# InternRobotics/InternNav

Hardware: AMD Instinct MI355X
Metric: policy steps/sec/node (higher is better)
Workload: dtype bf16

## Files before the change

internnav_amd/csrc/dit_rowchain.hip:

```cpp
#include <type_traits>
#include <utility>

#pragma clang diagnostic ignored "-Winline-asm"

#include "common.h"
#include "kernels.h"

namespace {

typedef float f32x16 __attribute__((ext_vector_type(16)));
typedef unsigned int u32x2 __attribute__((ext_vector_type(2)));
typedef unsigned int u32x4 __attribute__((ext_vector_type(4)));

constexpr int RC_NS = 4, RC_BN = 128, RC_STAGE = RC_BN * 64, RC_D = 384, RC_NT1 = RC_D / RC_BN, RC_KC2 = RC_D / 64;
constexpr size_t RC_LDS = size_t(RC_NS) * RC_STAGE * sizeof(bf16) + 2 * RC_D * sizeof(float);

__device__ __forceinline__ void rc_glds16(const void* base, uint32_t voff, uint32_t lds_byte_addr) {
    asm volatile("s_mov_b32 m0, %0\n\ts_nop 0\n\tglobal_load_lds_dwordx4 %1, %2" ::"s"(lds_byte_addr), "v"(voff), "s"(base) : "memory", "m0");
}

template <int N>
__device__ __forceinline__ void rc_wait_vm() {
    asm volatile("s_waitcnt vmcnt(%0)" ::"n"(N) : "memory");
}
// ... 356 lines not shown
                    for (int h = 0; h < 2; ++h) {
                        unsigned q[2][2];
#pragma unroll
                        for (int i = 0; i < 2; ++i) {
                            q[i][0] = rc_pack2(acc[j][(2 * h + i) * 4], acc[j][(2 * h + i) * 4 + 1]);
                            q[i][1] = rc_pack2(acc[j][(2 * h + i) * 4 + 2], acc[j][(2 * h + i) * 4 + 3]);
                        }
                        const u32x4 o = rc_merge_rows(q[0][0], q[0][1], q[1][0], q[1][1]);
                        *reinterpret_cast<u32x4*>(Cb + crow + nt * 128 + j * 32 + h * 16 + khalf * 8) = o;
                    }
                }
            }
        }
        rc_wait_vm<0>();
    }
}

template <int NW, int KC1, bool HAS2, bool GLU2>
int launch_rowchain(const ina_dit_rowchain_args& p, hipStream_t stream) {
    auto kern = dit_rowchain_kernel<NW, KC1, HAS2, GLU2>;
    static bool attr_done = false;
    if (!attr_done) {
        INA_HIP_CHECK(hipFuncSetAttribute(reinterpret_cast<const void*>(kern), hipFuncAttributeMaxDynamicSharedMemorySize, (int)RC_LDS));
        attr_done = true;
    }
    const double n2 = HAS2 ? (double)p.N2 : 0.0;
    InaProfScope prof(INA_PROF_GEMM, 2.0 * p.M * RC_D * (p.K1 + n2),
                      2.0 * p.M * p.K1 + 2.0 * RC_D * (p.K1 + n2) + 8.0 * p.M * RC_D + (p.H ? 2.0 * p.M * RC_D : 0.0) + 2.0 * p.M * (GLU2 ? n2 / 2 : n2), stream);
    hipLaunchKernelGGL(kern, dim3(p.M / (NW * 32)), dim3(NW * 64), RC_LDS, stream, p);
    INA_HIP_CHECK(hipGetLastError());
    return 0;
}

}

int ina_launch_dit_rowchain(const ina_dit_rowchain_args& p_in, hipStream_t stream) {
    ina_dit_rowchain_args p = p_in;
    if (p.mod_div <= 0) p.mod_div = p.M;
    constexpr int nw = 4;
    INA_REQUIRE(p.A && p.W1 && p.X && p.gamma1, "dit_rowchain: A, W1, X and gamma1 are required");
    INA_REQUIRE(p.K1 == 384 || p.K1 == 1024, "dit_rowchain: K1=%d (built for 384 = attn2.to_out and 1024 = feed_forward.linear_2)", p.K1);
    INA_REQUIRE(p.M > 0 && p.M % (nw * 32) == 0 && p.mod_div % (nw * 32) == 0, "dit_rowchain: M=%d and mod_div=%d must be multiples of the %d-row panel", p.M,
                p.mod_div, nw * 32);
    INA_REQUIRE(p.lda % 8 == 0 && p.ldw1 % 8 == 0 && p.ldx % 4 == 0 && (!p.H || p.ldh % 8 == 0), "dit_rowchain: row strides must keep 16-byte alignment");
    INA_REQUIRE(((uintptr_t)p.A % 16) == 0 && ((uintptr_t)p.W1 % 16) == 0 && ((uintptr_t)p.X % 16) == 0 && ((uintptr_t)p.H % 16) == 0, "dit_rowchain: misaligned pointer");
    INA_REQUIRE((!p.gate && !p.mod_scale2) || p.mod_ld >= RC_D, "dit_rowchain: modulation needs mod_ld >= 384");
    INA_REQUIRE((size_t)384 * p.ldw1 < (1u << 30) && (!p.W2 || (size_t)p.N2 * p.ldw2 < (1u << 30)), "dit_rowchain: weight too large for 32-bit element offsets");
    INA_REQUIRE(p.W2 || !p.seg_stats, "dit_rowchain: seg_stats are statistics of the second GEMM's output rows");
    if (p.W2) {
        INA_REQUIRE(p.C2 && p.N2 > 0 && p.N2 % 128 == 0 && p.ldw2 % 8 == 0 && p.ldc2 % 8 == 0 && ((uintptr_t)p.W2 % 16) == 0 && ((uintptr_t)p.C2 % 16) == 0,
                    "dit_rowchain: second GEMM needs C2, N2 %% 128 == 0 and 16-byte aligned rows (N2=%d)", p.N2);
        INA_REQUIRE(!p.seg_stats || (!p.glu2 && p.N2 % 384 == 0 && ((uintptr_t)p.seg_stats % 8) == 0), "dit_rowchain: seg_stats needs a plain second GEMM with N2 %% 384 == 0 (N2=%d)", p.N2);
        INA_REQUIRE(p.glu2 ? p.K1 == 384 : p.K1 != 384, "dit_rowchain: built pairs are (K1 = 384, SwiGLU second GEMM) and (K1 = 1024, plain second GEMM)");
    }
    ina_prof_set_sub(42);
    if (p.K1 == 384) return !p.W2 ? launch_rowchain<4, 6, false, false>(p, stream) : launch_rowchain<4, 6, true, true>(p, stream);
    return !p.W2 ? launch_rowchain<4, 16, false, false>(p, stream) : launch_rowchain<4, 16, true, false>(p, stream);
}
```

internnav_amd/nextdit.py:

```python
from __future__ import annotations

import math
from typing import Dict

import numpy as np
import torch

from . import ops
from .navdp import IMAGENET_MEAN, IMAGENET_STD, _DecoderLayer, _SeqWorkspace, decoder_layer_postnorm
from .vit_s import DinoV2Encoder, VitWorkspace


def _interleave16(a: torch.Tensor, b: torch.Tensor) -> torch.Tensor:
    n, k = a.shape
    return torch.stack([a.view(n // 16, 16, k), b.view(n // 16, 16, k)], dim=1).reshape(2 * n, k).contiguous()


class NextDiTSystem1:
    def __init__(self, state_dict: Dict[str, torch.Tensor], cfg: dict, device="cuda:0", max_envs: int = 64, use_async: bool = True, row_chain: bool = True):
        dev = torch.device(device)
        bf, f32 = torch.bfloat16, torch.float32
        sd = state_dict
        self.cfg, self.device, self.b_max = cfg, dev, max_envs
        self.row_chain = (bool(row_chain) and cfg["dit_dim"] == 384 and cfg["dit_ffn"] in (1024, 1536)
                          and (cfg["sample_num"] * cfg["predict_size"]) % 128 == 0)
        self.chain_min_rows = 16384
        self.chain_a, self.chain_b = True, cfg["dit_ffn"] <= 1024
        self.chain_stats = True
        D, L, S, T = cfg["dit_dim"], cfg["latent_dim"], cfg["sample_num"], cfg["predict_size"]
        self.D, self.L, self.S, self.T, self.nq = D, L, S, T, cfg["n_query"]
        self.Fr = cfg["memory_frames"]
        self.use_async = bool(use_async)
        self.Lz = (32 if self.use_async else 0) + self.nq
        self.nl, self.nh = cfg["dit_layers"], cfg["dit_heads"]

        def w(k):
            return sd[k].to(device=dev, dtype=bf).contiguous()

        def f(k):
            return sd[k].to(device=dev, dtype=f32).contiguous()

        self.cp = [(w("cond_projector.0.weight"), f("cond_projector.0.bias")), (w("cond_projector.2.weight"), f("cond_projector.2.bias"))]
        nm = self.Fr * 256
        self.nm = nm
        if self.use_async:
            self.vit = DinoV2Encoder(sd, "rgb_model.", dev)
            self.vit_ws = VitWorkspace(max_envs * self.Fr, dev)
            self.mem_pos = sd["memory_encoder.memory_pos"][:nm].to(device=dev, dtype=f32).contiguous()
        self.me_layers = []
        for i in range(3 if self.use_async else 0):
            p = f"memory_encoder.encoder.layers.{i}"
            self.me_layers.append(dict(sa_w=w(p + ".self_attn.in_proj_weight"), sa_b=f(p + ".self_attn.in_proj_bias"),
                                       sa_ow=w(p + ".self_attn.out_proj.weight"), sa_ob=f(p + ".self_attn.out_proj.bias"),
                                       l1w=w(p + ".linear1.weight"), l1b=f(p + ".linear1.bias"), l2w=w(p + ".linear2.weight"),
                                       l2b=f(p + ".linear2.bias"), n1=(f(p + ".norm1.weight"), f(p + ".norm1.bias")),
                                       n2=(f(p + ".norm2.weight"), f(p + ".norm2.bias"))))
        if self.use_async:
            self.me_ws = _SeqWorkspace(max_envs * nm, D, 2048, dev)
            self.memcat = torch.empty(max_envs * nm, L, dtype=bf, device=dev)
            self.q_layers = [_DecoderLayer(sd, f"rgb_resampler.decoder.layers.{i}", dev, L) for i in range(3)]
# ... 118 lines not shown
        rows = B * nq
        ops.linear(traj_latents.reshape(rows, -1), self.cp[0][0], bias=self.cp[0][1], act="gelu_tanh", out=self.cp_h[:rows])
        ops.linear(self.cp_h[:rows].view(B, nq, L), self.cp[1][0], bias=self.cp[1][1], out=z3[:, Lz - nq:, :], batched=True)
        if self.use_async and not images_encoded:
            self.encode_images(B, images_dp)
        self._derive_condition(B, cs)

    def _derive_condition(self, B: int, cs: dict):
        D, Lz = self.D, self.Lz
        zr = B * Lz
        ops.linear(cs["z"][:zr], self.cap[0][0], bias=self.cap[0][1], act="gelu_tanh", out=cs["cap_h"][:zr])
        ops.linear(cs["cap_h"][:zr], self.cap[1][0], bias=self.cap[1][1], out=cs["enc"][:zr])
        ops.pool_act(cs["enc"][:zr], cs["pool"][:B], T=Lz)
        ops.norm(cs["pool"][:B], self.ce_ln[0], self.ce_ln[1], eps=1e-5, out=cs["pool_n"][:B])
        ops.linear(cs["pool_n"][:B], self.ce_w, bias=self.ce_b, out=cs["cap_emb"][:B])
        for l, Lr in enumerate(self.layers):
            ops.norm(cs["enc"][:zr], Lr["ctx"], None, eps=1e-5, rms=True, out=cs["enc_n"][:zr])
            kv = cs["kv2"][l][:zr]
            ops.linear(cs["enc_n"][:zr], Lr["wkv2"], out=kv)
            kk = kv.view(zr * 2, D)
            ops.norm(kk, Lr["k2n"][0], Lr["k2n"][1], eps=1e-5, out=kk, rows=zr, in_map=(1, 2, 0), out_map=(1, 2, 0))
            ops.dit_v2t(kv.view(B, Lz, 2, self.nh, D // self.nh), self.nh, cs["v2t"][l])

    def _dit_layer(self, l: int, B: int, cs: dict = None, x_buf: torch.Tensor = None):
        Lr, D, S, T, Lz, nh = self.layers[l], self.D, self.S, self.T, self.Lz, self.nh
        cs = cs or self._cond_set()
        rows, nseq, hd = B * S * T, B * S, D // self.nh
        x, h, att, qkvq, proj, ff = (self.x if x_buf is None else x_buf)[:rows], self.h[:rows], self.att[:rows], self.qkvq[:rows], self.proj[:rows], self.ff[:rows]
        mod = cs["mod"]
        m = mod[:B, l * 4 * D:(l + 1) * 4 * D]
        scale_msa, gate_msa, scale_mlp, gate_mlp = m[:, :D], m[:, D:2 * D], m[:, 2 * D:3 * D], m[:, 3 * D:]
        chain = self.row_chain and rows >= self.chain_min_rows
        chain_a, chain_b = chain and self.chain_a, chain and self.chain_b
        stats = self.qstats[:rows] if (chain and self.chain_stats and D == 384) else None
        if l == 0 or not chain_b:
            if l == 0:
                ops.norm(x, Lr["n1"], None, eps=1e-5, rms=True, mod_scale=scale_msa, mod_div=S * T, out=h)
            ops.linear(h, Lr["wq"], out=qkvq, seg_stats=(stats, 1e-5) if stats is not None else None)
        kv5 = cs["kv2"][l][: B * Lz].view(B, Lz, 2, nh, hd)
        ops.dit_attention(qkvq, att, (Lr["q1n"], Lr["k1n"], Lr["q2n"]), kv5, cs["v2t"][l], Lr["gate"], T=T, seq_per_env=S, heads=nh, eps=1e-5, stats=stats)
        last = l + 1 >= self.nl
        nxt = None if last else mod[:B, (l + 1) * 4 * D:(l + 1) * 4 * D + D]
        if chain_a:
            ops.dit_rowchain(att, Lr["wo"], Lr["n2"], x, gate=gate_msa, gamma2=Lr["fn1"], mod_scale2=scale_mlp, w2=Lr["w13"], c2=ff, glu2=True,
                             mod_div=S * T, eps=1e-5)
        else:
            ops.linear(att, Lr["wo"], out=proj)
            ops.norm(proj, Lr["n2"], None, eps=1e-5, rms=True, gate=gate_msa, base=x, mod_div=S * T, out32=x,
                     out2=h, gamma2=Lr["fn1"], mod_scale2=scale_mlp)
            ops.linear(h, Lr["w13"], act="silu", glu=True, out=ff)
        if chain_b:
            if last:
                ops.dit_rowchain(ff, Lr["w2"], Lr["fn2"], x, gate=gate_mlp, mod_div=S * T, eps=1e-5)
            else:
                ops.dit_rowchain(ff, Lr["w2"], Lr["fn2"], x, gate=gate_mlp, gamma2=self.layers[l + 1]["n1"], mod_scale2=nxt,
                                 w2=self.layers[l + 1]["wq"], c2=qkvq, mod_div=S * T, eps=1e-5, seg_stats=stats, seg_eps=1e-5)
            return
        ops.linear(ff, Lr["w2"], out=proj)
        if last:
            ops.norm(proj, Lr["fn2"], None, eps=1e-5, rms=True, gate=gate_mlp, base=x, mod_div=S * T, out32=x)
        else:
            ops.norm(proj, Lr["fn2"], None, eps=1e-5, rms=True, gate=gate_mlp, base=x, mod_div=S * T, out32=x,
                     out2=h, gamma2=self.layers[l + 1]["n1"], mod_scale2=nxt)

    def generate_traj(self, traj_latents: torch.Tensor, images_dp: torch.Tensor, x_init: torch.Tensor, guidance_scale: float = 1.0,
                      images_encoded: bool = False) -> torch.Tensor:
        B = traj_latents.shape[0]
        assert B <= self.b_max and traj_latents.dtype == torch.bfloat16
        D, S, T = self.D, self.S, self.T
        rows = B * S * T
        cs = self._cond_set()
        self.encode_condition(B, traj_latents, images_dp, cs, images_encoded=images_encoded)
        cfg_on = float(guidance_scale) != 1.0
        sets = [(cs, self.x)]
        if cfg_on:
            from . import train_ops as Tr

            null = self._cond_set(null=True)
            self._derive_condition(B, null)
            sets.append((null, self.x_u))
        sample = self.sample[:rows]
        sample.copy_(x_init.reshape(rows, 3))
        nmod = self.nl * 4 * D
        if cfg_on:
            dts = torch.from_numpy(self.sigmas[1:] - self.sigmas[:-1]).float()
            g = float(guidance_scale)
            coefs = torch.stack([dts * g, dts * (1.0 - g)], 1)[:, :, None].expand(-1, -1, 3).contiguous().to(self.device)
        for i in range(self.cfg["num_inference_steps"]):
            dt = float(self.sigmas[i + 1] - self.sigmas[i])
# ... 17 lines not shown
```

internnav_amd/qwen_vl.py:

```python
from __future__ import annotations

import weakref
from types import SimpleNamespace
from typing import Dict, List, Optional, Sequence, Tuple

import numpy as np
import torch

from . import ops
from .runtime import CapacityError


def vision_window_permutation(grids: Sequence[Tuple[int, int, int]], merge: int = 2, window: int = 112, patch: int = 14):
    win = window // merge // patch
    idx_all, cu, base = [], [0], 0
    for t, h, w in grids:
        gh, gw = h // merge, w // merge
        idx = np.arange(t * gh * gw).reshape(t, gh, gw)
        ph, pw = win - gh % win, win - gw % win
        nh, nw = (gh + ph) // win, (gw + pw) // win
        pad = np.pad(idx, ((0, 0), (0, ph), (0, pw)), constant_values=-100)
        pad = pad.reshape(t, nh, win, nw, win).transpose(0, 1, 3, 2, 4).reshape(t, nh * nw, win * win)
        lens = (pad != -100).sum(-1).reshape(-1)
        flat = pad.reshape(-1)
# ... 21 lines not shown

def rope_index(input_ids: np.ndarray, grids, image_token_id: int, vision_start_id: int, merge: int = 2):
    B, S = input_ids.shape
    pos = np.zeros((3, B, S), dtype=np.int64)
    deltas = np.zeros(B, dtype=np.int64)
    img = 0
    for b in range(B):
        toks = input_ids[b]
        starts = np.nonzero((toks[:-1] == vision_start_id) & (toks[1:] == image_token_id))[0]
        chunks, st, nxt = [], 0, 0
        for s0 in starts:
            ed = int(s0) + 1
            t, h, w = grids[img]
            img += 1
            gh, gw = h // merge, w // merge
            text_len = ed - st
            chunks.append(np.broadcast_to(np.arange(text_len)[None], (3, text_len)) + nxt)
            ti = np.zeros(t * gh * gw, dtype=np.int64)
            hi = np.broadcast_to(np.arange(gh)[None, :, None], (t, gh, gw)).reshape(-1)
            wi = np.broadcast_to(np.arange(gw)[None, None, :], (t, gh, gw)).reshape(-1)
            vis = np.stack([ti, hi, wi]) + text_len + nxt
            chunks.append(vis)
            nxt = int(vis.max()) + 1
            st = ed + t * gh * gw
        if st < S:
            chunks.append(np.broadcast_to(np.arange(S - st)[None], (3, S - st)) + nxt)
        p = np.concatenate(chunks, axis=1)
        pos[:, b] = p
        deltas[b] = int(p.max()) + 1 - S
    return pos, deltas


SKINNY_GEMM_MAX_ROWS = 64
ATTN_WIDE_MIN_ROWS = 128


def kv_image_cut(ids: np.ndarray, n: int, image_token_id: int) -> int:
    while 0 < n < ids.shape[0] and ids[n - 1] == image_token_id and ids[n] == image_token_id:
        n -= 1
    return n


def kv_reuse_lengths(ids: np.ndarray, seq_lens, cached_ids: Sequence[Optional[np.ndarray]], image_token_id: int) -> np.ndarray:
    B, S = ids.shape
    lens = np.asarray(seq_lens, dtype=np.int64).reshape(B)
    pl = np.zeros(B, dtype=np.int64)
    for b in range(B):
        c = cached_ids[b]
        if c is None or len(c) == 0:
            continue
        m = min(len(c), int(lens[b]) - 1)
        diff = np.nonzero(ids[b, :m] != np.asarray(c[:m]))[0]
        n = int(diff[0]) if diff.size else m
        pl[b] = kv_image_cut(ids[b], n, image_token_id)
    need = max(ATTN_WIDE_MIN_ROWS, SKINNY_GEMM_MAX_ROWS // B + 1)
    if pl.any() and S - int(pl.min()) < need:
        b = int(np.argmin(pl))
        pl[b] = kv_image_cut(ids[b], max(0, min(int(pl[b]), S - need)), image_token_id)
    return pl


def kv_reuse_fit(pl: np.ndarray, S: int, tail: int, s_max: int) -> Tuple[np.ndarray, int]:
    pl = np.asarray(pl, dtype=np.int64).copy()
    dropped = 0
    while pl.any() and int(pl.max()) + S - int(pl.min()) + tail > s_max:
        pl[int(np.argmax(pl))] = 0
# ... 96 lines not shown
    for k in sd.keys():
        v = sd[k]
        if k in names:
            out[k] = ops.mx4_quantize(v.to(torch.bfloat16).contiguous())[2].to(v.dtype)
        elif k == "lm_head.weight":
            out[k] = ops.w8_quantize(v.to(torch.bfloat16).contiguous())[2].to(v.dtype)
        else:
            out[k] = v
    return out


def _interleave16(a: torch.Tensor, b: torch.Tensor) -> torch.Tensor:
    n, k = a.shape
    return torch.stack([a.view(n // 16, 16, k), b.view(n // 16, 16, k)], dim=1).reshape(2 * n, k).contiguous()


def _pad_rows(t: torch.Tensor, n: int) -> torch.Tensor:
    return t if t.shape[0] == n else torch.cat([t, t.new_zeros((n - t.shape[0],) + tuple(t.shape[1:]))], 0)


class QwenVLEngine:

    def __init__(self, weights, cfg: dict, device="cuda:0", max_seqs: int = 16, max_seq_len: int = 1024, max_patches: int = 16 * 3136,
                 frag_weights: Optional[bool] = None, w8_decode: bool = False, token_logprobs: bool = False, max_decode: int = 128,
                 mx4_decode: bool = False):
        if w8_decode and mx4_decode:
            raise ValueError("w8_decode and mx4_decode are two roundings of the same weights: choose one")
        dev = torch.device(device)
        bf, f32 = torch.bfloat16, torch.float32
        self.cfg, self.device = cfg, dev
        self.B_max, self.S_max, self.Np_max = max_seqs, max_seq_len, max_patches
        self.fuse_decode_norm = True
        self.split_prefill = True
        self.split_serial = False
        self._side = None
        self.fuse_decode_rope = True
        self.tap = None
        D, I = cfg["v_hidden"], cfg["v_inter"]
        Ip = (I + 63) // 64 * 64
        self.vD, self.vI, self.vH, self.vhd = D, Ip, cfg["v_heads"], D // cfg["v_heads"]
        H, TI = cfg["t_hidden"], cfg["t_inter"]
        self.H, self.TI, self.nh, self.nkv = H, TI, cfg["t_heads"], cfg["t_kv_heads"]
        self.hd = H // self.nh
        self.qkv_w = (self.nh + 2 * self.nkv) * self.hd
        self.kv_w = 2 * self.nkv * self.hd
        W = weights

        def w(k):
            return W[k].to(device=dev, dtype=bf).contiguous()

        def f(k):
            return W[k].to(device=dev, dtype=f32).contiguous()

        self.v_patch = W["visual.patch_embed.proj.weight"].to(device=dev, dtype=bf).reshape(D, -1).contiguous()
        self.v_blocks = []
        for i in range(cfg["v_depth"]):
            b = f"visual.blocks.{i}."
            gw_, uw = _pad_rows(W[b + "mlp.gate_proj.weight"].to(dev).float(), Ip), _pad_rows(W[b + "mlp.up_proj.weight"].to(dev).float(), Ip)
            gb, ub = _pad_rows(W[b + "mlp.gate_proj.bias"].to(dev).float(), Ip), _pad_rows(W[b + "mlp.up_proj.bias"].to(dev).float(), Ip)
            dw = W[b + "mlp.down_proj.weight"].to(dev).float()
            dw = torch.cat([dw, dw.new_zeros(D, Ip - I)], 1) if Ip != I else dw
            self.v_blocks.append(dict(
                n1=f(b + "norm1.weight"), n2=f(b + "norm2.weight"), qkv_w=w(b + "attn.qkv.weight"), qkv_b=f(b + "attn.qkv.bias"),
                proj_w=w(b + "attn.proj.weight"), proj_b=f(b + "attn.proj.bias"),
                gu_w=_interleave16(gw_, uw).to(bf), gu_b=_interleave16(gb[:, None], ub[:, None]).reshape(-1).contiguous(),
                down_w=dw.to(bf).contiguous(), down_b=f(b + "mlp.down_proj.bias"), full=i in cfg["v_fullatt"]))
# ... 206 lines not shown
        pos0 = np.broadcast_to(np.asarray(cache_pos0, dtype=np.int64).reshape(-1, 1), (B, 1))
        rows = ((b0 + np.arange(B))[:, None] * self.S_max + pos0 + np.arange(S)[None]).reshape(-1).astype(np.int32)
        if int(pos0.max()) + S > self.S_max:
            raise CapacityError(f"KV cache capacity exceeded: {int(pos0.max()) + S} tokens > max_seq_len={self.S_max}")
        ph = dict(B=B, S=S, pos=torch.from_numpy(np.ascontiguousarray(np.broadcast_to(pos3, (3, B, S)).reshape(3, B * S)).astype(np.int32)).to(dev),
                  rows=torch.from_numpy(rows).to(dev), Lk=int(pos0.max()) + S, k_len=None, b0=b0, r0=b0 * S)
        if k_len is not None:
            ph["k_len"] = torch.from_numpy(np.asarray(k_len, dtype=np.int32)).to(dev)
        ph["new_are_last"] = bool(np.all((np.asarray(k_len).reshape(-1) if k_len is not None else ph["Lk"]) == pos0[:, 0] + S))
        ph["w0"] = pos0[:, 0].copy()
        return ph

    def _layers(self, ph: dict):
        H, nh, nkv, hd, Smax = self.H, self.nh, self.nkv, self.hd, self.S_max
        B, S = ph["B"], ph["S"]
        rows, r0, b0 = B * S, ph.get("r0", 0), ph.get("b0", 0)
        if self._kv_views and "w0" in ph:
            self._kv_evict({b0 + i: int(w) for i, w in enumerate(ph["w0"])})
        x, h, att, qkv, ff, x_in, cos, sin = (t[r0:r0 + rows] for t in (self.x, self.h, self.att, self.qkv, self.ff, self.x_in, self.cos, self.sin))
        ops.mrope_table(ph["pos"], self.inv_freq, self.axis_of, cos, sin)
        q4 = qkv[:, : nh * hd].view(B, S, nh, hd)
        single = rows <= 16 and self.tap is None
        fused_norm = single and self.fuse_decode_norm
        pfx = ph.get("prefix")
        if pfx is not None:
            k4 = qkv[:, nh * hd:(nh + nkv) * hd].view(B, S, nkv, hd)
            v4 = qkv[:, (nh + nkv) * hd:].view(B, S, nkv, hd)
        shr = ph.get("shared")
        fuse_rope = pfx is None and shr is None and single and self.fuse_decode_rope and ph.get("new_are_last", False) and ops.attention_rope_ok(S, ph["Lk"], nh, nkv, hd)
        if fuse_rope:
            kn4 = qkv[:, nh * hd:(nh + nkv) * hd].view(B, S, nkv, hd)
            vn4 = qkv[:, (nh + nkv) * hd:].view(B, S, nkv, hd)
        quant = ("8" if self.w8_decode else "4" if self.mx4_decode else None) if rows <= SKINNY_GEMM_MAX_ROWS else None
        for li, L in enumerate(self.layers):
            src = x_in if li == 0 else x
            wf = (lambda k, L=L: L.get(k)) if (self.frag_weights and rows > SKINNY_GEMM_MAX_ROWS) else (lambda k: None)
            if fused_norm:
                self._linear(src, L, "qkv_w", quant, bias=L["qkv_b"], out=qkv, prenorm=(L["n1"], 1e-6))
            else:
                ops.norm(src, L["n1"], None, eps=1e-6, rms=True, out=h)
                self._linear(h, L, "qkv_w", quant, bias=L["qkv_b"], out=qkv, w_frag=wf("qkv_wf"))
            if pfx is not None:
                ops.rope(qkv, cos, sin, heads=nh + nkv, D=hd, col0=0, rows=rows)
                kvc = L["kv"].view(self.B_max, Smax, 2, nkv, hd)
                tl = pfx.get("tail")
                if tl is None:
                    ops.attention_prefix(q4, k4, v4, kvc[:, :, 0], kvc[:, :, 1], pfx["slot"], pfx["pfx_len"], pfx["suf_len"],
                                         out=att.view(B, S, nh, hd), max_pfx=pfx["max_pfx"])
                else:
                    t5 = tl["tails"][li][: tl["rows"] * tl["T"]].view(tl["rows"], tl["T"], 2, nkv, hd)
                    ops.attention_prefix_tail(q4, k4, v4, kvc[:, :, 0], kvc[:, :, 1], pfx["slot"], pfx["pfx_len"], pfx["suf_len"], t5[:, :, 0],
                                              t5[:, :, 1], tl["tail_row"], tl["tail_len"], out=att.view(B, S, nh, hd), max_pfx=pfx["max_pfx"],
                                              max_tail=tl["max_tail"])
            elif shr is not None:
                tail = shr["tails"][li]
                ops.rope(qkv, cos, sin, heads=nh + nkv, D=hd, col0=0, rows=rows, kv_out=tail, kv_dst=shr["kv_dst"], kv_head0=nh, v_heads=nkv)
                kvc = L["kv"].view(self.B_max, Smax, 2, nkv, hd)
                t5 = tail[: rows * shr["T"]].view(rows, shr["T"], 2, nkv, hd)
                ops.attention_shared(qkv[:, : nh * hd].view(rows, nh, hd), t5[:, :, 0], t5[:, :, 1], kvc[:, :, 0], kvc[:, :, 1], shr["tile_rows"],
                                     shr["tile_slot"], shr["tile_pfx"], shr["tail_len"], out=att.view(rows, nh, hd), max_pfx=shr["max_pfx"])
            else:
                if not fuse_rope:
                    ops.rope(qkv, cos, sin, heads=nh + nkv, D=hd, col0=0, rows=rows, kv_out=L["kv"], kv_dst=ph["rows"], kv_head0=nh, v_heads=nkv)
                kv4 = L["kv"].view(self.B_max, Smax, 2, nkv, hd)[b0:b0 + B, : ph["Lk"]]
                ops.attention(q4, kv4[:, :, 0], kv4[:, :, 1], causal=True, out=att.view(B, S, nh, hd), k_len=ph["k_len"],
                              rope=(cos, sin, kn4, vn4) if fuse_rope else None)
            self._linear(att, L, "o_w", quant, residual=src, out=x)
            if fused_norm:
                self._linear(x, L, "gu_w", quant, act="silu", glu=True, out=ff, prenorm=(L["n2"], 1e-6))
            else:
                ops.norm(x, L["n2"], None, eps=1e-6, rms=True, out=h)
                self._linear(h, L, "gu_w", quant, act="silu", glu=True, out=ff, w_frag=wf("gu_wf"))
            self._linear(ff, L, "down_w", quant, residual=x, out=x, w_frag=wf("down_wf"))
            if self.tap is not None:
                self.tap("llm", li, x)

    def _suffix_phase(self, slot, next_pos, pfx_len, suf_len, m: int, tail_row=None, tail_len=None) -> dict:
        dev = self.device
        slot, pfx_len, suf_len = (np.asarray(v, dtype=np.int64).reshape(-1) for v in (slot, pfx_len, suf_len))
        P = slot.size
        assert P >= 1 and pfx_len.size == P and suf_len.size == P and np.asarray(next_pos).size == P
        if not 1 <= m <= ops.ATTN_PREFIX_MAX_ROWS:
            raise ValueError(f"a suffix pass runs 1 .. {ops.ATTN_PREFIX_MAX_ROWS} tokens per pair, got {m}")
        if P * m > self.x.shape[0]:
            raise CapacityError(f"suffix pass of {P} x {m} tokens exceeds the engine's {self.x.shape[0]} buffer rows")
        assert int(slot.min()) >= 0 and int(slot.max()) < self.B_max and int(pfx_len.min()) >= 0 and int(pfx_len.max()) <= self.S_max
        assert int(suf_len.min()) >= 0 and int(suf_len.max()) <= m
        pos = (np.asarray(next_pos, dtype=np.int64).reshape(-1, 1) + np.arange(m)[None]).reshape(1, P * m)
        i32 = lambda v: torch.from_numpy(np.ascontiguousarray(v).astype(np.int32)).to(dev)
        prefix = dict(slot=i32(slot), pfx_len=i32(pfx_len), suf_len=i32(suf_len), max_pfx=int(pfx_len.max()))
        if tail_row is not None:
            bufs = self._shared
            tail_row, tail_len = (np.asarray(v, dtype=np.int64).reshape(-1) for v in (tail_row, tail_len))
            assert bufs is not None and tail_row.size == P and tail_len.size == P
            assert int(tail_row.min()) >= 0 and int(tail_row.max()) < bufs.rows and int(tail_len.min()) >= 0 and int(tail_len.max()) <= bufs.T
            prefix["tail"] = dict(tails=bufs.tails, rows=bufs.rows, T=bufs.T, tail_row=i32(tail_row), tail_len=i32(tail_len), max_tail=int(tail_len.max()))
        return dict(B=P, S=m, pos=i32(np.broadcast_to(pos, (3, P * m))), b0=0, r0=0, prefix=prefix)

    def suffix_pass(self, state: dict, prompt_of, tokens, suf_len) -> torch.Tensor:
        tokens = np.asarray(tokens, dtype=np.int64)
        P, m = tokens.shape
        prompt_of = np.asarray(prompt_of, dtype=np.int64).reshape(-1)
        assert prompt_of.size == P and int(prompt_of.min()) >= 0 and int(prompt_of.max()) < state["B"]
        lens = state.get("lens")
        pl = np.full(state["B"], state["S"], dtype=np.int64) if lens is None else np.asarray(lens, dtype=np.int64)
        ph = self._suffix_phase(prompt_of, np.asarray(state["next_pos"])[prompt_of], pl[prompt_of], suf_len, m)
        ops.gather_rows(self.embed, self.x_in, src=torch.from_numpy(tokens.reshape(-1).astype(np.int32)).to(self.device), rows=P * m)
        self._layers(ph)
# ... 168 lines not shown
                    P["cached"].append((c, torch.from_numpy(img_pos[off[k]:off[k + 1]]).to(dev)))
        traj_pos = np.nonzero(flat == cfg["traj_token_id"])[0].astype(np.int32)
        if traj_pos.size:
            nq = self.latent_q.shape[0]
            P["traj_src"] = torch.from_numpy((np.arange(traj_pos.size) % nq).astype(np.int32)).to(dev)
            P["traj_dst"] = torch.from_numpy(traj_pos).to(dev)
        pos3, _ = rope_index(ids, grids_all, cfg["image_token_id"], cfg["vision_start_id"])
        if int(pl.max()) == 0:
            P["prefill"] = self._phase(B, Sr, pos3, 0)
            info = P.pop("_split_info", None)
            if self.split_prefill and B >= 2 and info is not None:
                img_seq, ntok, off, img_pos = info
                P["split"] = []
                Ba = (B + 1) // 2
                for b0, b1 in ((0, Ba), (Ba, B)):
                    ks = [k for k in range(len(grids_all)) if b0 <= img_seq[k] < b1]
                    if not ks or ks != list(range(ks[0], ks[-1] + 1)):
                        P.pop("split")
                        break
                    vp = self.plan_vision([grids_all[k] for k in ks])
                    vp["p0"] = int(sum(t * h * w for t, h, w in grids_all[: ks[0]]))
                    P["split"].append(dict(vision=vp, img_src=torch.from_numpy(vp["inv"]).to(dev), tok0=int(off[ks[0]]), n_tok=int(off[ks[-1] + 1] - off[ks[0]]),
                                           img_dst=torch.from_numpy(np.concatenate([img_pos[off[k]:off[k + 1]] for k in ks])).to(dev),
                                           prefill=self._phase(b1 - b0, Sr, pos3[:, b0:b1], 0, b0=b0)))
        P.pop("_split_info", None)
        if int(pl.max()) != 0:
            pos_run = np.zeros((3, B, Sr), dtype=np.int64)
            for b in range(B):
                n = S - pl[b]
                pos_run[:, b, :n] = pos3[:, b, pl[b]:]
                pos_run[:, b, n:] = pos3[:, b, -1:]
            uniform = bool((pl == pl[0]).all())
            P["prefill"] = self._phase(B, Sr, pos_run, pl, k_len=None if uniform else pl + Sr)
        nxt = pos3[:, :, -1].max(axis=0) + 1
        P["next_pos"] = nxt
        P["decode"] = [self._phase(B, 1, (nxt + j)[None, :, None], S + j) for j in range(max(n_decode - 1, 0))]
        if with_latents:
            nq = self.latent_q.shape[0]
            cur = S + max(n_decode - 1, 0)
            m = 1 if n_decode > 0 else 0
            p = (nxt + (cur - S))[None, :, None] + np.arange(m + nq)[None, None, :]
            P["latents"] = self._phase(B, m + nq, p, cur)
            P["lat_m"] = m
        return P

    def run_prefill(self, P: dict, pixel_values: Optional[torch.Tensor]):
        if self._kv_views:
            self._kv_evict({b: int(w) for b, w in enumerate(P["prefill"]["w0"])})
        ops.gather_rows(self.embed, self.x_in, src=P["ids"])
        if self.split_prefill and P.get("split") and self.tap is None:
            if "traj_src" in P:
                ops.gather_rows(self.latent_q, self.x_in, src=P["traj_src"], dst=P["traj_dst"])
            main = torch.cuda.current_stream()
            if self._side is None:
                self._side = torch.cuda.Stream(device=self.device)
            self._side.wait_stream(main)

            def half(s):
                vp = s["vision"]
                emb = self.run_vision(vp, pixel_values[vp["p0"]: vp["p0"] + vp["Np"]])
                tok = self.emb_tok[s["tok0"]: s["tok0"] + s["n_tok"]]
                ops.gather_rows(emb, tok, src=s["img_src"])
                ops.gather_rows(tok, self.x_in, dst=s["img_dst"])
                self._layers(s["prefill"])

            with ops.shared_tail():
# ... 354 lines not shown
```

Baseline: 299.1.

## Add small-M rowchain kernel and compute only tail rows in last prefill layer

Adds a 64-row-panel fused GEMM+RMSNorm+residual kernel for DiT layers below the large-row threshold (and K1=1536), replacing separate linear+norm launches in the non-chained path. Separately, the Qwen-VL prefill's final layer now runs attention and MLP only for the last 128 tokens per sequence, scattering the final row back. This avoids computing the full last layer for positions whose output is not consumed. It adds layout constraints and relies on only the last token's hidden state being needed downstream.

```diff
diff --git a/internnav_amd/csrc/dit_rowchain.hip b/internnav_amd/csrc/dit_rowchain.hip
--- a/internnav_amd/csrc/dit_rowchain.hip
+++ b/internnav_amd/csrc/dit_rowchain.hip
@@ -412,16 +412,214 @@
     return 0;
 }
 
+template <int KW, int NS>
+struct RcSmall {
+    static constexpr int ROWS = 64, SROWS = ROWS + RC_D, PR = KW / 8, RPI = 64 / PR, INST = SROWS / RPI / 4, NA = ROWS / RPI, STAGE = SROWS * KW;
+    static constexpr size_t LDS = size_t(NS) * STAGE * sizeof(bf16) + 2 * RC_D * sizeof(float) + 2 * 4 * ROWS * sizeof(float);
+    static_assert(KW == 64 && (NS == 2 || NS == 4) && INST * 4 * RPI == SROWS, "128-byte stage rows (the swizzle below); pieces must deal out evenly");
+    __device__ static constexpr int swz(int r) { return (r >> 1) & 7; }
+};
+
+template <int KW, int NS>
+__global__ __launch_bounds__(256) void dit_rowchain_small_kernel(ina_dit_rowchain_args p) {
+    using G = RcSmall<KW, NS>;
+    constexpr int D = RC_D, STAGE = G::STAGE, INST = G::INST, KS = KW / 16;
+    extern __shared__ __attribute__((aligned(1024))) char smem_raw[];
+    bf16* Ws = reinterpret_cast<bf16*>(smem_raw);
+    float* tab = reinterpret_cast<float*>(Ws + NS * STAGE);
+    float* red = tab + 2 * D;
+    const int tid = threadIdx.x, lane = tid & 63;
+    const int wave = __builtin_amdgcn_readfirstlane(tid >> 6);
+    const int mwg = blockIdx.x * G::ROWS;
+    const int lrow = lane & 31, khalf = lane >> 5;
+    const int total = p.K1 / KW;
+    const bf16* __restrict__ Ablk = reinterpret_cast<const bf16*>(p.A) + (size_t)mwg * p.lda;
+    const bf16* __restrict__ W1 = reinterpret_cast<const bf16*>(p.W1);
+    const uint32_t lds0 = (uint32_t)(uintptr_t)(__attribute__((address_space(3))) char*)smem_raw;
+    uint32_t voff[INST];
+    {
+        const int drow = lane / G::PR, dcp = lane % G::PR;
+#pragma unroll
+        for (int s = 0; s < INST; ++s) {
+            const int q = wave * INST + s, sr = q * G::RPI + drow, ch = (dcp ^ G::swz(sr)) << 3;
+            voff[s] = (uint32_t)(q < G::NA ? sr * p.lda + ch : (sr - G::ROWS) * p.ldw1 + ch) * 2u;
+        }
+    }
+    auto issue = [&](int st) {
+        const int s2 = st < total ? st : total - 1;
+        const uint32_t dst = lds0 + ((st & (NS - 1)) * STAGE * 2 + wave * INST * 1024);
+        const bf16* ab = Ablk + s2 * KW;
+        const bf16* wb = W1 + s2 * KW;
+#pragma unroll
+        for (int s = 0; s < INST; ++s) rc_glds16(wave * INST + s < G::NA ? ab : wb, voff[s], __builtin_amdgcn_readfirstlane(dst + s * 1024u));
+    };
+    int foff[KS];
+#pragma unroll
+    for (int kk = 0; kk < KS; ++kk) foff[kk] = lrow * KW + (((kk * 2 + khalf) ^ G::swz(lrow)) << 3);
+    const int wrow0 = G::ROWS + wave * 96;
+
+    f32x16 acc[2][3];
+#pragma unroll
+    for (int rb = 0; rb < 2; ++rb)
+#pragma unroll
+        for (int cb = 0; cb < 3; ++cb)
+#pragma unroll
+            for (int r = 0; r < 16; ++r) acc[rb][cb][r] = 0.f;
+#pragma unroll
+    for (int s = 0; s < NS - 1; ++s) issue(s);
+    {
+        const int mb = mwg / p.mod_div;
+        const float* gt = p.gate ? p.gate + (size_t)mb * p.mod_ld : nullptr;
+        const float* ms = p.mod_scale2 ? p.mod_scale2 + (size_t)mb * p.mod_ld : nullptr;
+        for (int i = tid; i < D; i += 256) {
+            tab[i] = gt ? p.gamma1[i] * tanhf(gt[i]) : p.gamma1[i];
+            const float g2 = p.gamma2 ? p.gamma2[i] : 1.0f;
+            tab[D + i] = ms ? g2 * (1.0f + ms[i]) : g2;
+        }
+    }
+    for (int t = 0; t < total; ++t) {
+        rc_wait_vm<(NS - 2) * INST>();
+        __builtin_amdgcn_s_barrier();
+        issue(t + NS - 1);
+        __builtin_amdgcn_sched_barrier(0);
+        const bf16* st = Ws + (t & (NS - 1)) * STAGE;
+        bf16x8 af[2][2], wf[2][3];
+#pragma unroll
+        for (int rb = 0; rb < 2; ++rb) af[0][rb] = *reinterpret_cast<const bf16x8*>(st + rb * 32 * KW + foff[0]);
+#pragma unroll
+        for (int cb = 0; cb < 3; ++cb) wf[0][cb] = *reinterpret_cast<const bf16x8*>(st + (wrow0 + cb * 32) * KW + foff[0]);
+#pragma unroll
+        for (int kk = 0; kk < KS; ++kk) {
+            if (kk + 1 < KS) {
+#pragma unroll
+                for (int rb = 0; rb < 2; ++rb) af[(kk + 1) & 1][rb] = *reinterpret_cast<const bf16x8*>(st + rb * 32 * KW + foff[kk + 1]);
+#pragma unroll
+                for (int cb = 0; cb < 3; ++cb) wf[(kk + 1) & 1][cb] = *reinterpret_cast<const bf16x8*>(st + (wrow0 + cb * 32) * KW + foff[kk + 1]);
+            }
+            __builtin_amdgcn_sched_barrier(0);
+#pragma unroll
+            for (int rb = 0; rb < 2; ++rb)
+#pragma unroll
+                for (int cb = 0; cb < 3; ++cb) acc[rb][cb] = __builtin_amdgcn_mfma_f32_32x32x16_bf16(wf[kk & 1][cb], af[kk & 1][rb], acc[rb][cb], 0, 0, 0);
+            __builtin_amdgcn_sched_barrier(0);
+        }
+        asm volatile("s_waitcnt lgkmcnt(0)" ::: "memory");
+    }
+
+    auto row_sums = [&](int which, float (&s)[2]) {
+#pragma unroll
+        for (int rb = 0; rb < 2; ++rb) {
+            s[rb] += __shfl_xor(s[rb], 32);
+            red[(which * 4 + wave) * G::ROWS + rb * 32 + lrow] = s[rb];
+        }
+        __syncthreads();
+#pragma unroll
+        for (int rb = 0; rb < 2; ++rb) {
+            const float* r = red + which * 4 * G::ROWS + rb * 32 + lrow;
+            s[rb] = ((r[0] + r[G::ROWS]) + r[2 * G::ROWS]) + r[3 * G::ROWS];
+        }
+    };
+    float s1[2] = {0.f, 0.f};
+#pragma unroll
+    for (int rb = 0; rb < 2; ++rb)
+#pragma unroll
+        for (int cb = 0; cb < 3; ++cb)
+#pragma unroll
+            for (int r = 0; r < 16; r += 2) {
+                const unsigned u = rc_pack2(acc[rb][cb][r], acc[rb][cb][r + 1]);
+                const float a = rc_lo(u), b = rc_hi(u);
+                acc[rb][cb][r] = a;
+                acc[rb][cb][r + 1] = b;
+                s1[rb] += a * a;
+                s1[rb] += b * b;
+            }
+    row_sums(0, s1);
+    float s2[2] = {0.f, 0.f};
+#pragma unroll
+    for (int rb = 0; rb < 2; ++rb) {
+        const float rstd1 = rsqrtf(s1[rb] * (1.0f / D) + p.eps);
+        float* xrow = p.X + (size_t)(mwg + rb * 32 + lrow) * p.ldx + wave * 96 + khalf * 4;
+#pragma unroll
+        for (int cb = 0; cb < 3; ++cb) {
+            f32x4 xv[4];
+#pragma unroll
+            for (int i = 0; i < 4; ++i) xv[i] = *reinterpret_cast<const f32x4*>(xrow + cb * 32 + i * 8);
+#pragma unroll
+            for (int i = 0; i < 4; ++i) {
+                const f32x4 gg = *reinterpret_cast<const f32x4*>(tab + wave * 96 + cb * 32 + i * 8 + khalf * 4);
+                f32x4 o;
+#pragma unroll
+                for (int e = 0; e < 4; ++e) {
+                    float w = acc[rb][cb][i * 4 + e] * rstd1;
+                    w *= gg[e];
+                    w += xv[i][e];
+                    o[e] = w;
+                    acc[rb][cb][i * 4 + e] = w;
+                    s2[rb] += w * w;
+                }
+                *reinterpret_cast<f32x4*>(xrow + cb * 32 + i * 8) = o;
+            }
+        }
+    }
+    if (p.H) {
+        row_sums(1, s2);
+#pragma unroll
+        for (int rb = 0; rb < 2; ++rb) {
+            const float rstd2 = rsqrtf(s2[rb] * (1.0f / D) + p.eps);
+            bf16* hrow = reinterpret_cast<bf16*>(p.H) + (size_t)(mwg + rb * 32 + lrow) * p.ldh + wave * 96 + khalf * 8;
+#pragma unroll
+            for (int cb = 0; cb < 3; ++cb)
+#pragma unroll
+                for (int m = 0; m < 2; ++m) {
+                    unsigned q[2][2];
+#pragma unroll
+                    for (int h = 0; h < 2; ++h) {
+                        const int i = 2 * m + h;
+                        const f32x4 hh = *reinterpret_cast<const f32x4*>(tab + D + wave * 96 + cb * 32 + i * 8 + khalf * 4);
+                        float w[4];
+#pragma unroll
+                        for (int e = 0; e < 4; ++e) {
+                            w[e] = acc[rb][cb][i * 4 + e] * rstd2;
+                            w[e] *= hh[e];
+                        }
+                        q[h][0] = rc_pack2(w[0], w[1]);
+                        q[h][1] = rc_pack2(w[2], w[3]);
+                    }
+                    *reinterpret_cast<u32x4*>(hrow + cb * 32 + m * 16) = rc_merge_rows(q[0][0], q[0][1], q[1][0], q[1][1]);
+                }
+        }
+    }
+    rc_wait_vm<0>();
+}
+
+template <int KW, int NS>
+int launch_rowchain_small(const ina_dit_rowchain_args& p, hipStream_t stream) {
+    using G = RcSmall<KW, NS>;
+    auto kern = dit_rowchain_small_kernel<KW, NS>;
+    static bool attr_done = false;
+    if (!attr_done) {
+        INA_HIP_CHECK(hipFuncSetAttribute(reinterpret_cast<const void*>(kern), hipFuncAttributeMaxDynamicSharedMemorySize, (int)G::LDS));
+        attr_done = true;
+    }
+    InaProfScope prof(INA_PROF_GEMM, 2.0 * p.M * RC_D * p.K1,
+                      2.0 * p.M * p.K1 + 2.0 * RC_D * p.K1 + 8.0 * p.M * RC_D + (p.H ? 2.0 * p.M * RC_D : 0.0), stream);
+    hipLaunchKernelGGL(kern, dim3(p.M / G::ROWS), dim3(256), G::LDS, stream, p);
+    INA_HIP_CHECK(hipGetLastError());
+    return 0;
+}
+
 }
 
 int ina_launch_dit_rowchain(const ina_dit_rowchain_args& p_in, hipStream_t stream) {
     ina_dit_rowchain_args p = p_in;
     if (p.mod_div <= 0) p.mod_div = p.M;
-    constexpr int nw = 4;
+    const bool small = !p.W2 && (p.M < 16384 || p.K1 == 1536);
+    const int panel = small ? 64 : 128;
     INA_REQUIRE(p.A && p.W1 && p.X && p.gamma1, "dit_rowchain: A, W1, X and gamma1 are required");
-    INA_REQUIRE(p.K1 == 384 || p.K1 == 1024, "dit_rowchain: K1=%d (built for 384 = attn2.to_out and 1024 = feed_forward.linear_2)", p.K1);
-    INA_REQUIRE(p.M > 0 && p.M % (nw * 32) == 0 && p.mod_div % (nw * 32) == 0, "dit_rowchain: M=%d and mod_div=%d must be multiples of the %d-row panel", p.M,
-                p.mod_div, nw * 32);
+    INA_REQUIRE(p.K1 == 384 || p.K1 == 1024 || (p.K1 == 1536 && !p.W2),
+                "dit_rowchain: K1=%d (built for 384 = attn2.to_out and 1024 = feed_forward.linear_2; 1536 without a second GEMM only)", p.K1);
+    INA_REQUIRE(p.M > 0 && p.M % panel == 0 && p.mod_div % panel == 0, "dit_rowchain: M=%d and mod_div=%d must be multiples of the %d-row panel", p.M,
+                p.mod_div, panel);
     INA_REQUIRE(p.lda % 8 == 0 && p.ldw1 % 8 == 0 && p.ldx % 4 == 0 && (!p.H || p.ldh % 8 == 0), "dit_rowchain: row strides must keep 16-byte alignment");
     INA_REQUIRE(((uintptr_t)p.A % 16) == 0 && ((uintptr_t)p.W1 % 16) == 0 && ((uintptr_t)p.X % 16) == 0 && ((uintptr_t)p.H % 16) == 0, "dit_rowchain: misaligned pointer");
     INA_REQUIRE((!p.gate && !p.mod_scale2) || p.mod_ld >= RC_D, "dit_rowchain: modulation needs mod_ld >= 384");
@@ -434,6 +632,10 @@
         INA_REQUIRE(p.glu2 ? p.K1 == 384 : p.K1 != 384, "dit_rowchain: built pairs are (K1 = 384, SwiGLU second GEMM) and (K1 = 1024, plain second GEMM)");
     }
     ina_prof_set_sub(42);
+    if (small) {
+        INA_REQUIRE((size_t)64 * p.lda < (1u << 30), "dit_rowchain: A row stride too large for 32-bit element offsets");
+        return launch_rowchain_small<64, 2>(p, stream);
+    }
     if (p.K1 == 384) return !p.W2 ? launch_rowchain<4, 6, false, false>(p, stream) : launch_rowchain<4, 6, true, true>(p, stream);
     return !p.W2 ? launch_rowchain<4, 16, false, false>(p, stream) : launch_rowchain<4, 16, true, false>(p, stream);
 }
diff --git a/internnav_amd/nextdit.py b/internnav_amd/nextdit.py
--- a/internnav_amd/nextdit.py
+++ b/internnav_amd/nextdit.py
@@ -26,6 +26,9 @@
                           and (cfg["sample_num"] * cfg["predict_size"]) % 128 == 0)
         self.chain_min_rows = 16384
         self.chain_a, self.chain_b = True, cfg["dit_ffn"] <= 1024
+        self.small_chain = (bool(row_chain) and cfg["dit_dim"] == 384 and cfg["dit_ffn"] in (1024, 1536)
+                            and (cfg["sample_num"] * cfg["predict_size"]) % 64 == 0)
+        self.small_a, self.small_b = True, cfg["dit_ffn"] <= 1024
         self.chain_stats = True
         D, L, S, T = cfg["dit_dim"], cfg["latent_dim"], cfg["sample_num"], cfg["predict_size"]
         self.D, self.L, self.S, self.T, self.nq = D, L, S, T, cfg["n_query"]
@@ -210,6 +213,7 @@
         scale_msa, gate_msa, scale_mlp, gate_mlp = m[:, :D], m[:, D:2 * D], m[:, 2 * D:3 * D], m[:, 3 * D:]
         chain = self.row_chain and rows >= self.chain_min_rows
         chain_a, chain_b = chain and self.chain_a, chain and self.chain_b
+        small = self.small_chain and rows < self.chain_min_rows
         stats = self.qstats[:rows] if (chain and self.chain_stats and D == 384) else None
         if l == 0 or not chain_b:
             if l == 0:
@@ -223,9 +227,12 @@
             ops.dit_rowchain(att, Lr["wo"], Lr["n2"], x, gate=gate_msa, gamma2=Lr["fn1"], mod_scale2=scale_mlp, w2=Lr["w13"], c2=ff, glu2=True,
                              mod_div=S * T, eps=1e-5)
         else:
-            ops.linear(att, Lr["wo"], out=proj)
-            ops.norm(proj, Lr["n2"], None, eps=1e-5, rms=True, gate=gate_msa, base=x, mod_div=S * T, out32=x,
-                     out2=h, gamma2=Lr["fn1"], mod_scale2=scale_mlp)
+            if small and self.small_a:
+                ops.dit_rowchain(att, Lr["wo"], Lr["n2"], x, gate=gate_msa, gamma2=Lr["fn1"], mod_scale2=scale_mlp, h=h, mod_div=S * T, eps=1e-5)
+            else:
+                ops.linear(att, Lr["wo"], out=proj)
+                ops.norm(proj, Lr["n2"], None, eps=1e-5, rms=True, gate=gate_msa, base=x, mod_div=S * T, out32=x,
+                         out2=h, gamma2=Lr["fn1"], mod_scale2=scale_mlp)
             ops.linear(h, Lr["w13"], act="silu", glu=True, out=ff)
         if chain_b:
             if last:
@@ -233,6 +240,12 @@
             else:
                 ops.dit_rowchain(ff, Lr["w2"], Lr["fn2"], x, gate=gate_mlp, gamma2=self.layers[l + 1]["n1"], mod_scale2=nxt,
                                  w2=self.layers[l + 1]["wq"], c2=qkvq, mod_div=S * T, eps=1e-5, seg_stats=stats, seg_eps=1e-5)
+            return
+        if small and self.small_b:
+            if last:
+                ops.dit_rowchain(ff, Lr["w2"], Lr["fn2"], x, gate=gate_mlp, mod_div=S * T, eps=1e-5)
+            else:
+                ops.dit_rowchain(ff, Lr["w2"], Lr["fn2"], x, gate=gate_mlp, gamma2=self.layers[l + 1]["n1"], mod_scale2=nxt, h=h, mod_div=S * T, eps=1e-5)
             return
         ops.linear(ff, Lr["w2"], out=proj)
         if last:
diff --git a/internnav_amd/qwen_vl.py b/internnav_amd/qwen_vl.py
--- a/internnav_amd/qwen_vl.py
+++ b/internnav_amd/qwen_vl.py
@@ -77,6 +77,7 @@
 
 
 SKINNY_GEMM_MAX_ROWS = 64
+TAIL_ROWS = 128
 ATTN_WIDE_MIN_ROWS = 128
 
 
@@ -239,6 +240,8 @@
         self.B_max, self.S_max, self.Np_max = max_seqs, max_seq_len, max_patches
         self.fuse_decode_norm = True
         self.split_prefill = True
+        self.prefill_tail_only = True
+        self.x_tail = None
         self.split_serial = False
         self._side = None
         self.fuse_decode_rope = True
@@ -511,6 +514,7 @@
             kn4 = qkv[:, nh * hd:(nh + nkv) * hd].view(B, S, nkv, hd)
             vn4 = qkv[:, (nh + nkv) * hd:].view(B, S, nkv, hd)
         quant = ("8" if self.w8_decode else "4" if self.mx4_decode else None) if rows <= SKINNY_GEMM_MAX_ROWS else None
+        tail = ph.get("tail") if (self.prefill_tail_only and self.tap is None and pfx is None and shr is None and len(self.layers) > 1) else None
         for li, L in enumerate(self.layers):
             src = x_in if li == 0 else x
             wf = (lambda k, L=L: L.get(k)) if (self.frag_weights and rows > SKINNY_GEMM_MAX_ROWS) else (lambda k: None)
@@ -542,6 +546,9 @@
                 if not fuse_rope:
                     ops.rope(qkv, cos, sin, heads=nh + nkv, D=hd, col0=0, rows=rows, kv_out=L["kv"], kv_dst=ph["rows"], kv_head0=nh, v_heads=nkv)
                 kv4 = L["kv"].view(self.B_max, Smax, 2, nkv, hd)[b0:b0 + B, : ph["Lk"]]
+                if tail is not None and li == len(self.layers) - 1:
+                    self._layer_tail(ph, L, q4, kv4, x, h, att, ff, wf)
+                    break
                 ops.attention(q4, kv4[:, :, 0], kv4[:, :, 1], causal=True, out=att.view(B, S, nh, hd), k_len=ph["k_len"],
                               rope=(cos, sin, kn4, vn4) if fuse_rope else None)
             self._linear(att, L, "o_w", quant, residual=src, out=x)
@@ -553,6 +560,27 @@
             self._linear(ff, L, "down_w", quant, residual=x, out=x, w_frag=wf("down_wf"))
             if self.tap is not None:
                 self.tap("llm", li, x)
+
+    def _mark_tail(self, ph: dict):
+        B, S, T = ph["B"], ph["S"], TAIL_ROWS
+        assert S >= T
+        b = np.arange(B, dtype=np.int64)
+        i32 = lambda v: torch.from_numpy(np.ascontiguousarray(v).astype(np.int32)).to(self.device)
+        ph["tail"] = dict(src=i32((b[:, None] * S + (S - T) + np.arange(T)[None]).reshape(-1)), last_src=i32(b * T + T - 1), last_dst=i32(b * S + S - 1))
+        if self.x_tail is None:
+            self.x_tail = torch.empty(self.B_max * T, self.H, dtype=self.x.dtype, device=self.device)
+
+    def _layer_tail(self, ph: dict, L: dict, q4, kv4, x, h, att, ff, wf):
+        B, S, T, nh, hd = ph["B"], ph["S"], TAIL_ROWS, self.nh, self.hd
+        t, n = ph["tail"], B * TAIL_ROWS
+        xt = self.x_tail[ph.get("b0", 0) * T: ph.get("b0", 0) * T + n]
+        ops.attention(q4[:, S - T:], kv4[:, :, 0], kv4[:, :, 1], causal=True, out=att[:n].view(B, T, nh, hd), k_len=ph["k_len"])
+        ops.gather_rows(x, xt, src=t["src"])
+        ops.linear(att[:n], L["o_w"], residual=xt, out=xt)
+        ops.norm(xt, L["n2"], None, eps=1e-6, rms=True, out=h[:n])
+        ops.linear(h[:n], L["gu_w"], act="silu", glu=True, out=ff[:n], w_frag=wf("gu_wf"))
+        ops.linear(ff[:n], L["down_w"], residual=xt, out=xt, w_frag=wf("down_wf"))
+        ops.gather_rows(xt, x, src=t["last_src"], dst=t["last_dst"])
 
     def _suffix_phase(self, slot, next_pos, pfx_len, suf_len, m: int, tail_row=None, tail_len=None) -> dict:
         dev = self.device
@@ -787,6 +815,10 @@
                 pos_run[:, b, n:] = pos3[:, b, -1:]
             uniform = bool((pl == pl[0]).all())
             P["prefill"] = self._phase(B, Sr, pos_run, pl, k_len=None if uniform else pl + Sr)
+        one_len = seq_lens is None or bool((np.asarray(seq_lens).reshape(-1) == S).all())
+        if (n_decode > 0 or with_latents) and one_len and Sr >= TAIL_ROWS and P["prefill"]["k_len"] is None:
+            for ph in [P["prefill"]] + [s["prefill"] for s in P.get("split", [])]:
+                self._mark_tail(ph)
         nxt = pos3[:, :, -1].max(axis=0) + 1
         P["next_pos"] = nxt
         P["decode"] = [self._phase(B, 1, (nxt + j)[None, :, None], S + j) for j in range(max(n_decode - 1, 0))]
```

Result: no change. 301.6 (median of 6 runs) (+0.8%).
